# Axionis47/semantic-search-kd

Hardware: AMD Instinct MI355X
Metric: docs embedded/sec + queries/sec@top-10 (1M×384-d corpus), 1→8 MI355X (higher is better)
Workload: dtype bf16 screen + f32 exact; 1 GPU; cosine top-10: 10000 queries x 1000000 x 384-d fp32 corpus in HBM (configs[1] search), row-sharded over 1 GPU(s), all-gather + merge; corpus_rows=1000000, queries=10000, k=10, queries_per_block=160, corpus_passes=63, slices=4, exact_fallback_queries=0, index_bytes=1536000000, sidecar_bytes=768004096, workspace_bytes=697277184

## Files before the change

include/sskd_amd.h:

```cpp
#ifndef SSKD_AMD_H
#define SSKD_AMD_H

#include <stddef.h>
#include <stdint.h>

#ifdef __cplusplus
extern "C" {
#endif

#define SSKD_ABI_VERSION 1

#define SSKD_OK 0
#define SSKD_ERR_INVALID 1
#define SSKD_ERR_WORKSPACE 2
#define SSKD_ERR_HIP 3
#define SSKD_ERR_UNSUPPORTED 4

#define SSKD_DIM 384
#define SSKD_TILE_ROWS 32
#define SSKD_K_PASS 32
#define SSKD_K_MAX 1024

int sskd_abi_version(void);
const char* sskd_last_error(void);
// ... 37 lines not shown

size_t sskd_index_bf16_bytes(int64_t n_rows);
int sskd_index_make_bf16(const float* d_tiled, int64_t n_rows, void* d_bf16, void* stream);
size_t sskd_index_search_screened_workspace_bytes(int64_t n_rows, int nq, int k);
int sskd_index_search_screened_plan(int64_t n_rows, int nq, int k, int* queries_per_block, int* corpus_passes,
                                    int* n_slices);
int sskd_index_search_screened(const float* d_tiled, const void* d_bf16, int64_t n_rows, const float* d_queries,
                               int nq, int k, int64_t id_offset, float* d_out_scores, int64_t* d_out_ids,
                               int* d_status, void* d_workspace, size_t workspace_bytes, void* stream,
                               void* ev_scan_begin, void* ev_scan_end);

size_t sskd_index_screen_band_scratch_bytes(int nq);
int sskd_index_screen_band(const void* d_bf16, int64_t n_rows, const float* d_queries, int nq, float* d_eps2_out,
                           void* d_scratch, size_t scratch_bytes, void* stream);

int sskd_index_screen_scores(const void* d_bf16, int64_t n_rows, const float* d_queries, int nq, float* d_out, void* stream);
int sskd_screen_threshold_roundtrip(const float* d_in, int n, float* d_out, void* stream);

int sskd_index_search_screened_plan_claims(int64_t n_rows, int nq, int k, int* claims);
int sskd_index_search_screened_claim(const float* d_tiled, const void* d_bf16, int64_t n_rows, const float* d_queries,
                                     int nq, int k, int64_t id_offset, const uint32_t* d_row_mask, int claim,
                                     float* d_out_scores, int64_t* d_out_ids, int* d_status, void* d_workspace,
                                     size_t workspace_bytes, void* stream, void* ev_scan_begin, void* ev_scan_end);

size_t sskd_index_search_onepass_workspace_bytes(int64_t n_rows, int nq, int k);
int sskd_index_search_onepass(const float* d_tiled, int64_t n_rows, const float* d_queries, int nq,
                              int k, int64_t id_offset, float* d_out_scores, int64_t* d_out_ids,
                              int* d_inexact, void* d_workspace, size_t workspace_bytes,
                              void* stream);

int64_t sskd_row_mask_words(int64_t n_rows);
int sskd_row_mask_pack(const uint8_t* d_flags, int64_t n_rows, uint32_t* d_mask, void* stream);
int sskd_row_mask_update(uint32_t* d_mask, int64_t n_rows, const int64_t* d_rows, int64_t n_ids, int allow,
                         int* d_bad, void* stream);
int sskd_row_mask_and(const uint32_t* d_a, const uint32_t* d_b, int64_t n_rows, uint32_t* d_out, void* stream);
int sskd_row_mask_count(const uint32_t* d_mask, int64_t n_rows, int64_t* d_count, void* stream);

int sskd_index_search_filtered(const float* d_tiled, int64_t n_rows, const float* d_queries, int nq, int k,
                               int64_t id_offset, const uint32_t* d_row_mask, float* d_out_scores,
                               int64_t* d_out_ids, void* d_workspace, size_t workspace_bytes, void* stream,
                               const sskd_search_tuning* tuning, void* ev_scan_begin, void* ev_scan_end);
int sskd_index_search_screened_filtered(const float* d_tiled, const void* d_bf16, int64_t n_rows, const float* d_queries,
                                        int nq, int k, int64_t id_offset, const uint32_t* d_row_mask, float* d_out_scores,
                                        int64_t* d_out_ids, int* d_status, void* d_workspace, size_t workspace_bytes,
                                        void* stream, void* ev_scan_begin, void* ev_scan_end);
int sskd_index_search_onepass_filtered(const float* d_tiled, int64_t n_rows, const float* d_queries, int nq,
// ... 387 lines not shown
```

semantic-search-kd_amd/_native.py:

```python
from __future__ import annotations

import ctypes as C
from pathlib import Path
from typing import Optional

_LIB_PATH = Path(__file__).resolve().parent / "libsskd_amd.so"

SSKD_OK = 0
SSKD_DIM = 384
SSKD_TILE_ROWS = 32
SSKD_K_PASS = 32
SSKD_K_MAX = 1024

_ERR_NAMES = {1: "INVALID", 2: "WORKSPACE", 3: "HIP", 4: "UNSUPPORTED"}


class NativeError(RuntimeError):

    def __init__(self, code: int, message: str):
        super().__init__(f"sskd_amd[{_ERR_NAMES.get(code, code)}]: {message}")
        self.code = code


class EncoderConfig(C.Structure):
# ... 95 lines not shown
    "sskd_index_search": (_i, [_vp, _i64, _vp, _i, _i, _i64, _vp, _vp, _vp, _sz, _vp]),
    "sskd_index_search_profiled": (_i, [_vp, _i64, _vp, _i, _i, _i64, _vp, _vp, _vp, _sz, _vp, _vp, _vp]),
    "sskd_index_search_plan": (_i, [_i64, _i, _i, _ip, _ip, _ip, _ip, _ip]),
    "sskd_index_search_workspace_bytes_ex": (_sz, [_i64, _i, _i, C.POINTER(SearchTuning)]),
    "sskd_index_search_ex": (
        _i, [_vp, _i64, _vp, _i, _i, _i64, _vp, _vp, _vp, _sz, _vp, C.POINTER(SearchTuning), _vp, _vp]
    ),
    "sskd_index_search_plan_ex": (_i, [_i64, _i, _i, C.POINTER(SearchTuning), _ip, _ip, _ip, _ip, _ip]),
    "sskd_topk_record_bytes": (_sz, [_i, _i]),
    "sskd_topk_merge_packed": (_i, [_vp, _i, _i, _i, _i, _vp, _vp, _vp]),
    "sskd_index_bf16_bytes": (_sz, [_i64]),
    "sskd_index_make_bf16": (_i, [_vp, _i64, _vp, _vp]),
    "sskd_index_search_screened_workspace_bytes": (_sz, [_i64, _i, _i]),
    "sskd_index_search_screened_plan": (_i, [_i64, _i, _i, _ip, _ip, _ip]),
    "sskd_index_search_screened": (_i, [_vp, _vp, _i64, _vp, _i, _i, _i64, _vp, _vp, _vp, _vp, _sz, _vp, _vp, _vp]),
    "sskd_index_search_screened_plan_claims": (_i, [_i64, _i, _i, _ip]),
    "sskd_index_search_screened_claim": (
        _i, [_vp, _vp, _i64, _vp, _i, _i, _i64, _vp, _i, _vp, _vp, _vp, _vp, _sz, _vp, _vp, _vp]
    ),
    "sskd_index_screen_band_scratch_bytes": (_sz, [_i]),
    "sskd_index_screen_band": (_i, [_vp, _i64, _vp, _i, _vp, _vp, _sz, _vp]),
    "sskd_index_screen_scores": (_i, [_vp, _i64, _vp, _i, _vp, _vp]),
    "sskd_screen_threshold_roundtrip": (_i, [_vp, _i, _vp, _vp]),
    "sskd_index_search_onepass_workspace_bytes": (_sz, [_i64, _i, _i]),
    "sskd_index_search_onepass": (_i, [_vp, _i64, _vp, _i, _i, _i64, _vp, _vp, _vp, _vp, _sz, _vp]),
    "sskd_row_mask_words": (_i64, [_i64]),
    "sskd_row_mask_pack": (_i, [_vp, _i64, _vp, _vp]),
    "sskd_row_mask_update": (_i, [_vp, _i64, _vp, _i64, _i, _vp, _vp]),
    "sskd_row_mask_and": (_i, [_vp, _vp, _i64, _vp, _vp]),
    "sskd_row_mask_count": (_i, [_vp, _i64, _vp, _vp]),
    "sskd_index_search_filtered": (
        _i, [_vp, _i64, _vp, _i, _i, _i64, _vp, _vp, _vp, _vp, _sz, _vp, C.POINTER(SearchTuning), _vp, _vp]
    ),
    "sskd_index_search_screened_filtered": (
        _i, [_vp, _vp, _i64, _vp, _i, _i, _i64, _vp, _vp, _vp, _vp, _vp, _sz, _vp, _vp, _vp]
    ),
    "sskd_index_search_onepass_filtered": (_i, [_vp, _i64, _vp, _i, _i, _i64, _vp, _vp, _vp, _vp, _vp, _sz, _vp]),
    "sskd_index_range_search_workspace_bytes": (_sz, [_i64, _i, _i64]),
    "sskd_index_range_search": (_i, [_vp, _i64, _vp, _i, _vp, _i64, _vp, _vp, _vp, _vp, _i64, _vp, _sz, _vp]),
    "sskd_range_record_bytes": (_sz, [_i, _i64]),
    "sskd_range_merge_workspace_bytes": (_sz, [_i, _i, _i64]),
    "sskd_range_merge_packed": (_i, [_vp, _i, _i, _i64, _vp, _vp, _vp, _i64, _vp, _sz, _vp]),
    "sskd_index_search_grouped_workspace_bytes": (_sz, [_i64, _i, _i, _i]),
    "sskd_index_search_grouped": (
        _i, [_vp, _i64, _vp, _i, _i, _i, _i64, _vp, _vp, _vp, _vp, _vp, _vp, _vp, _vp, _vp, _sz, _vp]
    ),
# ... 188 lines not shown
```

semantic-search-kd_amd/csrc/screen.hip:

```cpp
#include "search_device.h"
#include "search_host.h"

#include <algorithm>
#include <cfloat>

using sskd::require_shard_rows;

namespace {

typedef __bf16 sbf16x8 __attribute__((ext_vector_type(8)));
typedef float f32x4 __attribute__((ext_vector_type(4)));
constexpr int BSTEPS = DIM / 32;
constexpr int BTILE_VEC = 2 * BSTEPS * 64;
#ifndef SSKD_SCREEN_BGROUP
#define SSKD_SCREEN_BGROUP 3
#endif
#ifndef SSKD_SCREEN_WAVES
#define SSKD_SCREEN_WAVES 12
#endif
#ifndef SSKD_SCREEN_RING
#define SSKD_SCREEN_RING 2
#endif
constexpr int BGROUP = SSKD_SCREEN_BGROUP;
constexpr int SCREEN_RING = SSKD_SCREEN_RING;
#ifndef SSKD_SCREEN_BGROUP_Q5
#define SSKD_SCREEN_BGROUP_Q5 1
#endif
#ifndef SSKD_SCREEN_RING_Q5
#define SSKD_SCREEN_RING_Q5 3
#endif
constexpr int BGROUP_Q5 = SSKD_SCREEN_BGROUP_Q5, SCREEN_RING_Q5 = SSKD_SCREEN_RING_Q5;
#ifndef SSKD_SCREEN_TAU_REFRESH_TILES
#define SSKD_SCREEN_TAU_REFRESH_TILES 64
#endif
constexpr int SCREEN_TAU_REFRESH_TILES = SSKD_SCREEN_TAU_REFRESH_TILES;
#ifndef SSKD_SCREEN_BOUND_REFRESH_TILES
#define SSKD_SCREEN_BOUND_REFRESH_TILES 8
#endif
constexpr int SCREEN_BOUND_REFRESH_TILES = SSKD_SCREEN_BOUND_REFRESH_TILES;
constexpr int SCREEN_WAVES = SSKD_SCREEN_WAVES;
template <int BG, int RG>
struct ScreenRingOk {
  static_assert(BSTEPS % BG == 0 && (BSTEPS / BG) % RG == 0 && RG >= 2, "screening prefetch geometry");
  static constexpr bool value = true;
};
static_assert(ScreenRingOk<BGROUP, SCREEN_RING>::value && ScreenRingOk<BGROUP_Q5, SCREEN_RING_Q5>::value, "");
constexpr float SCREEN_ACC_SLACK = 1.0e-4f;
constexpr int SCREEN_MAX_CAND = 256;
constexpr int SCREEN_FALLBACK_TIER1 = 1024;
constexpr int SCREEN_LIGHT_MAX_TILES_PER_WAVE = 330;
constexpr int SCREEN_CUS = 256;

__global__ __launch_bounds__(256) void tile_colsum_kernel(const float4* __restrict__ tiled, int64_t n_tiles,
                                                          float* __restrict__ colsum) {
  const int c = threadIdx.x % CHUNKS, g = threadIdx.x / CHUNKS;
  if (g >= 2) return;
  float4 a = make_float4(0.f, 0.f, 0.f, 0.f);
  for (int64_t t = blockIdx.x; t < n_tiles; t += gridDim.x) {
// ... 46 lines not shown
    }
    out[t * BTILE_VEC + v] = o;
    atomicAdd(&rowss[0][r], nn);
    atomicAdd(&rowss[1][r], bb);
    atomicAdd(&rowss[2][r], dd);
    atomicMax(&amax, am);
  }
  __syncthreads();
  if (threadIdx.x < 96) {
    const float v = rowss[threadIdx.x >> 5][threadIdx.x & 31];
    atomicMax(norm_block + (threadIdx.x >> 5), __float_as_int(v < INFINITY ? v : INFINITY));
  }
  if (threadIdx.x == 96) atomicMax(norm_block + SIDECAR_ABSMAX_WORD, amax);
}

constexpr float SCREEN_MIN_CORPUS = 0x1p-40f, SCREEN_MIN_QUERY = 0x1p-96f;
constexpr float SCREEN_MIN_BAND = 0x1p-100f, SCREEN_MAX_BAND = 0x1p+100f;
__global__ __launch_bounds__(256) void screen_setup_kernel(const float* __restrict__ queries, int nq,
                                                           const int* __restrict__ max_norm2, float* __restrict__ eps2,
                                                           int* __restrict__ tau, int* __restrict__ fb_count,
                                                           int* __restrict__ d_status, int* __restrict__ cursors,
                                                           int n_cursors) {
  for (int i = blockIdx.x * 256 + threadIdx.x; i < n_cursors; i += gridDim.x * 256) cursors[i] = 0;
  if (threadIdx.x < 44) {
    const int64_t i = (int64_t)blockIdx.x * 44 + threadIdx.x;
    if (i < (int64_t)nq * 11) tau[i] = (int)0x80000000;
  }
  if (blockIdx.x == 0) {
    if (threadIdx.x < 64) fb_count[threadIdx.x] = 0;
    if (threadIdx.x < 2) d_status[threadIdx.x] = 0;
  }
  const int lane = threadIdx.x & 63;
  const int q = blockIdx.x * 4 + (threadIdx.x >> 6);
  if (q >= nq) return;
  float xs[DIM / 64];
  int am = 0;
#pragma unroll
  for (int i = 0; i < DIM / 64; ++i) {
    xs[i] = queries[(int64_t)q * DIM + lane + 64 * i];
    am = max(am, __float_as_int(xs[i]) & 0x7fffffff);
  }
#pragma unroll
  for (int o = 32; o > 0; o >>= 1) am = max(am, __shfl_xor(am, o));
  const int ex = min(max(am >> 23, 1), 253);
  const float down = __int_as_float(ex << 23), up = __int_as_float((254 - ex) << 23);
  float ss = 0.f, dd = 0.f;
#pragma unroll
  for (int i = 0; i < DIM / 64; ++i) {
    const float x = xs[i];
// ... 230 lines not shown
      for (int nb = 0; nb < 2 * QB; ++nb)
#pragma unroll
        for (int i = 0; i < 4; ++i) acc[mb][nb][i] = 0.f;
    screen_tile_groups<QB, 0, BG, RG, SCREEN_FRAG_DEPTH, NB>(buf, tiled + (int64_t)t * BTILE_VEC, qbase, qfrag, acc,
                                                             t + 1 < n_tiles, (int64_t)BTILE_VEC, lane_off);
#pragma unroll
    for (int mb = 0; mb < 2; ++mb)
#pragma unroll
      for (int nb = 0; nb < 2 * QB; ++nb)
#pragma unroll
        for (int i = 0; i < 4; ++i)
          out[(int64_t)(t * TILE_ROWS + 16 * mb + 4 * g + i) * (32 * QB) + 16 * nb + n] = acc[mb][nb][i];
  }
}

__global__ __launch_bounds__(256) void screen_thr_probe_kernel(const float* __restrict__ in, int n, float* __restrict__ out) {
  const int i = blockIdx.x * 256 + threadIdx.x;
  if (i >= n) return;
  const float x = in[i], y = (i ^ 1) < n ? in[i ^ 1] : -INFINITY;
  const unsigned packed = (i & 1) ? screen_thr_pack2(y, x) : screen_thr_pack2(x, y);
  out[i] = screen_thr_unpack(packed, i & 1);
}

template <int QB>
__device__ __forceinline__ void apply_tile_mask16(f32x4 (&acc)[2][2 * QB], uint32_t word, int g) {
  if (word == 0xFFFFFFFFu) return;
  const uint32_t lw = word >> (4 * g);
#pragma unroll
  for (int mb = 0; mb < 2; ++mb)
#pragma unroll
    for (int i = 0; i < 4; ++i) {
      const bool off = ((lw >> (16 * mb + i)) & 1u) == 0u;
#pragma unroll
      for (int nb = 0; nb < 2 * QB; ++nb)
        if (off) acc[mb][nb][i] = -INFINITY;
    }
}

template <int K, int QB, int WAVES, bool BOUND_ONLY, bool LIGHT, int BG, int RG, bool MASKED = false>
__device__ __forceinline__ void screen_tiles(const ScreenAppendParams& p, int t_begin, int t_end, int slice, int* cursors,
                                             int wave, int n, int g, int q0,
                                             const sbf16x8* __restrict__ qlane, int* pool, int list0,
                                             bool ragged, unsigned (&gthr)[QB]) {
  constexpr int NQ = 2 * QB;
  int* const wthr = pool + QB * 32 * K;
  float* const bandl = reinterpret_cast<float*>(wthr + QB * 32);
  short* const cnts = reinterpret_cast<short*>(bandl + QB * 32);
  sbf16x8 buf[RG][BG][2];
  constexpr int NB = screen_frag_bases<QB>();
  screen_lds_frag* qbase[NB];
#pragma unroll
  for (int nb = 0; nb < NB; ++nb) {
    qbase[nb] = (screen_lds_frag*)qlane + nb * SCREEN_FRAGS_PER_BASE * 64;
    asm volatile("" : "+v"(qbase[nb]));
  }
  sbf16x8 qfrag[SCREEN_FRAG_DEPTH];
#ifdef SSKD_SCREEN_ABL_CONTIG
  const unsigned lane_off = (unsigned)(n + 16 * g) * 16u;
#else
// ... 37 lines not shown
      c_end = next_end;
    }
  }
  if (t >= 0) {
#pragma unroll
    for (int gr = 0; gr + 1 < RG; ++gr) load_bgroup<BG>(buf[gr], p.tiled + (int64_t)t * BTILE_VEC + gr * BG * 128, lane_off);
  }

  for (int tiles_done = 0; t >= 0; t = next_t, ++tiles_done) {
    if (dealt) {
      next_t = t + WAVES < t_end ? t + WAVES : -1;
    } else {
      const int rem = c_end - t;
      if (rem == 2) draw();
      next_t = t + 1;
      if (rem == 1) {
        next_t = drawn_chunk();
        c_end = next_end;
      }
    }
    const sbf16x8* tile = p.tiled + (int64_t)t * BTILE_VEC;
    uint32_t mword = 0xFFFFFFFFu;
    if constexpr (MASKED) mword = tile_mask_word(p.row_mask, t);
    const bool exchange = !BOUND_ONLY && (tiles_done == 0 || tiles_done == 16 || tiles_done % SCREEN_TAU_REFRESH_TILES == 0);
    if (exchange || tiles_done % SCREEN_BOUND_REFRESH_TILES == 0) {
    const int lh = screen_lane_now(), nh = lh & 15;
    if (exchange && lh < 16) {
#pragma unroll
      for (int nb = 0; nb < NQ; ++nb) {
        const int ql = 16 * nb + nh;
        if (q0 + ql < p.nq) atomicMax(wthr + ql, exchange_bound<K>(p.gpool, p.tau + q0 + ql, q0 + ql, wthr[ql]));
      }
    }
#pragma unroll
    for (int pr = 0; pr < QB; ++pr) {
      float thr[2];
#pragma unroll
      for (int e = 0; e < 2; ++e) {
        const int nb = 2 * pr + e, ql = 16 * nb + nh;
        const int w = wthr[ql];
        const float bd = bandl[ql];
        thr[e] = ordered_to_float(w) - bd;
        thr[e] = fmaxf(thr[e], -INFINITY);
      }
      screen_thr_raise2(gthr[pr], thr[0], thr[1]);
      asm volatile("" : "+v"(gthr[pr]));
    }
    }
    f32x4 acc[2][NQ];
#pragma unroll
    for (int mb = 0; mb < 2; ++mb)
#pragma unroll
      for (int nb = 0; nb < NQ; ++nb)
#pragma unroll
        for (int i = 0; i < 4; ++i) acc[mb][nb][i] = 0.f;

// ... 29 lines not shown
      for (int e = 0; e < 2; ++e) {
        const int nb = 2 * pr + e;
        m[e] = acc[0][nb][0];
#pragma unroll
        for (int r = 1; r < 8; ++r) m[e] = fmaxf(m[e], acc[r >> 2][nb][r & 3]);
        fthr[e] = fmaxf(screen_thr_unpack(gthr[pr], e), -FLT_MAX);
        pass[e] = m[e] >= fthr[e];
      }
      if constexpr (BOUND_ONLY) {
#pragma unroll
        for (int e = 0; e < 2; ++e) {
          const int nb = 2 * pr + e;
          const float mg = screen_group_max(pass[e] ? m[e] : -INFINITY);
          if (pass[e]) {
            int nc = n;
            asm volatile("" : "+v"(nc));
            const int ql = 16 * nb + nc;
            if (m[e] == mg) {
              int xid = rowbase;
#pragma unroll
              for (int r = 7; r >= 0; --r) xid = acc[r >> 2][nb][r & 3] == m[e] ? rowbase + 16 * (r >> 2) + (r & 3) : xid;
              const int xi = float_to_ordered(m[e]);
              if (pool_offer<K>(pool + ql * K, wthr + ql, xi)) {
                bucket_forward<K>(p.gpool, q0 + ql, xid, xi);
              }
            }
            screen_thr_raise(gthr[pr], e, fmaxf(ordered_to_float(wthr[ql]) - bandl[ql], -INFINITY));
          }
        }
      } else
      if (__any(pass[0] || pass[1])) {
        const int lc = screen_lane_now(), nc = lc & 15, gc = lc >> 4;
        float pb[2];
        int c[2];
#pragma unroll
        for (int e = 0; e < 2; ++e) {
          const int ql = 32 * pr + 16 * e + nc;
          pb[e] = fmaxf(ordered_to_float(wthr[ql]) - bandl[ql], -INFINITY);
          c[e] = cnts[(ql * WAVES + wave) * 4 + gc];
        }
        screen_thr_raise2(gthr[pr], pb[0], pb[1]);
        const float thr[2] = {fmaxf(pb[0], fthr[0]), fmaxf(pb[1], fthr[1])};
        const auto run_of = [&](int ql) {
          return reinterpret_cast<unsigned long long*>(
              p.cand + ((int64_t)min(q0 + ql, p.nq - 1) * p.lists_per_query + list0 + gc) * SCREEN_CAP);
        };
        const auto compact_if_tight = [&](int ql, int& cc, float bound) {
#ifndef SSKD_SCREEN_NO_COMPACT
          const bool tight = cc > SCREEN_CAP - 8 && cc <= SCREEN_CAP;
          if (__any(tight)) {
            __builtin_amdgcn_s_waitcnt(0x0F70);
            if (tight) cc = screen_compact_run(run_of(ql), cc, bound);
          }
          return tight;
#else
          return false;
#endif
        };
        if constexpr (LIGHT) {
#pragma unroll
// ... 2 lines not shown
            if (!__any(m[e] >= thr[e])) continue;
            unsigned long long* const run = run_of(ql);
            int cc = c[e];
            const bool dirty = compact_if_tight(ql, cc, thr[e]);
            bool grew = false;
#pragma unroll
            for (int r = 0; r < 8; ++r) {
              const float x = acc[r >> 2][nb][r & 3];
              const int xid = rowbase + 16 * (r >> 2) + (r & 3);
              if (x >= thr[e]) {
                if (cc < SCREEN_CAP)
                  run[cc] = (unsigned long long)__float_as_uint(x) | ((unsigned long long)(unsigned)xid << 32);
                if (cc <= SCREEN_CAP) ++cc;
                grew = true;
              }
            }
            if (grew || dirty) cnts[(ql * WAVES + wave) * 4 + gc] = (short)cc;
            const float mg = screen_group_max(m[e]);
            if (grew && m[e] == mg) {
              int xid = rowbase;
#pragma unroll
              for (int r = 7; r >= 0; --r) xid = acc[r >> 2][nb][r & 3] == m[e] ? rowbase + 16 * (r >> 2) + (r & 3) : xid;
              const int xi = float_to_ordered(m[e]);
              if (pool_offer<K>(pool + ql * K, wthr + ql, xi) && tiles_done > 0)
                bucket_forward<K>(p.gpool, q0 + ql, xid, xi);
            }
          }
        } else {
          unsigned take = 0;
#pragma unroll
          for (int b = 15; b >= 0; --b)
            take = (take << 1) | (acc[(b >> 2) & 1][2 * pr + (b >> 3)][b & 3] >= thr[b >> 3] ? 1u : 0u);
          if (!__any(take != 0)) continue;
          int cc[2] = {c[0], c[1]};
          bool dirty[2] = {false, false};
#pragma unroll
          for (int e = 0; e < 2; ++e)
            if (__any((take >> (8 * e) & 0xFFu) != 0)) dirty[e] = compact_if_tight(32 * pr + 16 * e + nc, cc[e], thr[e]);
#pragma clang loop unroll(disable)
          for (unsigned rest = take; rest != 0; rest &= rest - 1) {
            const int b = __builtin_ctz(rest);
            const int e = b >> 3;
            const bool b0 = b & 1, b1 = b & 2, b2 = b & 4, b3 = b & 8;
            const auto &a0 = acc[0][2 * pr], &a1 = acc[1][2 * pr], &a2 = acc[0][2 * pr + 1], &a3 = acc[1][2 * pr + 1];
            const float x00 = b0 ? a0[1] : a0[0], x01 = b0 ? a0[3] : a0[2], x02 = b0 ? a1[1] : a1[0], x03 = b0 ? a1[3] : a1[2];
            const float x04 = b0 ? a2[1] : a2[0], x05 = b0 ? a2[3] : a2[2], x06 = b0 ? a3[1] : a3[0], x07 = b0 ? a3[3] : a3[2];
            const float x10 = b1 ? x01 : x00, x11 = b1 ? x03 : x02, x12 = b1 ? x05 : x04, x13 = b1 ? x07 : x06;
            const float x20 = b2 ? x11 : x10, x21 = b2 ? x13 : x12;
            const float x = b3 ? x21 : x20;
            const int xid = rowbase + 4 * (b & 4) + (b & 3);
            const int ql = 32 * pr + 16 * e + nc;
            int cn = e ? cc[1] : cc[0];
            if (cn < SCREEN_CAP) run_of(ql)[cn] = (unsigned long long)__float_as_uint(x) | ((unsigned long long)(unsigned)xid << 32);
            if (cn <= SCREEN_CAP) ++cn;
            cc[0] = e ? cc[0] : cn;
            cc[1] = e ? cn : cc[1];
            if (tiles_done > 0) {
              const int xi = float_to_ordered(x);
              if (pool_offer<K>(pool + ql * K, wthr + ql, xi))
                bucket_forward<K>(p.gpool, q0 + ql, xid, xi);
            }
          }
#pragma unroll
          for (int e = 0; e < 2; ++e) {
            const int ql = 32 * pr + 16 * e + nc;
            if (!__any((take >> (8 * e) & 0xFFu) != 0)) continue;
            const bool grew = (take >> (8 * e) & 0xFFu) != 0;
            if (grew || dirty[e]) cnts[(ql * WAVES + wave) * 4 + gc] = (short)cc[e];
            if (tiles_done == 0) {
              const float mg = screen_group_max(m[e]);
              if (grew && m[e] == mg) pool_offer<K>(pool + ql * K, wthr + ql, float_to_ordered(m[e]));
            }
          }
        }
      }
    }
  }

}

constexpr size_t screen_lds_bytes(int QB, int WAVES) {
  return (size_t)2 * QB * BSTEPS * 64 * 16 + (size_t)QB * 32 * (10 + 2) * sizeof(int) + (size_t)QB * 32 * WAVES * 4 * sizeof(short);
}
static_assert(screen_lds_bytes(5, SCREEN_WAVES) <= 160 * 1024, "the 160-query workgroup must fit the CU's LDS");

template <int K, int QB, int WAVES, bool LIGHT, int BG, int RG, bool MASKED = false>
__global__ __launch_bounds__(WAVES * 64) void screen_append_kernel(ScreenAppendParams p) {
  static_assert(K == 10, "screen_lds_bytes counts ten pool slots per query");
  extern __shared__ float4 qs_raw[];
  sbf16x8* const qs = reinterpret_cast<sbf16x8*>(qs_raw);
  const int tid = threadIdx.x;
  const int lane = tid & 63;
  const int wave = __builtin_amdgcn_readfirstlane(tid >> 6);
  const int n = lane & 15, g = lane >> 4;
// ... 14 lines not shown
  float* const bandl = reinterpret_cast<float*>(wthr + QB * 32);
  short* const cnts = reinterpret_cast<short*>(bandl + QB * 32);
  for (int i = tid; i < QB * 32 * (K + 1); i += WAVES * 64) pool[i] = (int)0x80000000;
  for (int i = tid; i < QB * 32; i += WAVES * 64) bandl[i] = p.eps2[min(q0 + i, p.nq - 1)];
  for (int i = tid; i < QB * 32 * WAVES * 2; i += WAVES * 64) reinterpret_cast<int*>(cnts)[i] = 0;
  __syncthreads();
  const sbf16x8* qlane = qs + lane;

  unsigned gthr[QB];
#pragma unroll
  for (int pr = 0; pr < QB; ++pr)
    gthr[pr] = (q0 + 32 * pr + n < p.nq ? 0xFC00u : 0x7C00u) | (q0 + 32 * pr + 16 + n < p.nq ? 0xFC000000u : 0x7C000000u);
  const int list0 = (slice * WAVES + wave) * 4;

  const bool ragged = (p.n_rows & 31) != 0;

  const int t_begin = slice * p.tiles_per_slice;
  const int t_end = min(t_begin + p.tiles_per_slice, p.n_tiles);
  if (p.pre_tps > 0) {
    const int s_begin = slice * p.pre_tps;
    const int s_end = min(s_begin + p.pre_tps, p.pre_tiles);
    screen_tiles<K, QB, WAVES, true, LIGHT, BG, RG, MASKED>(p, s_begin, s_end, slice, nullptr, wave, n, g, q0, qlane,
                                             pool, list0, ragged, gthr);
#pragma unroll
    for (int nb = 0; nb < 2 * QB; ++nb)
      if (g == 0 && q0 + nb * 16 + n < p.nq) atomicMax(p.tau + q0 + nb * 16 + n, wthr[nb * 16 + n]);
    __syncthreads();
    if ((SCREEN_STEAL && p.claim) || (s_begin < t_end && t_begin < s_end)) {
      for (int i = tid; i < QB * 32 * K; i += WAVES * 64) pool[i] = (int)0x80000000;
      __syncthreads();
    }
  }
#ifdef SSKD_SCREEN_STAMPS
  if (lane == 0) stamp[1] = __builtin_amdgcn_s_memrealtime();
#endif
  screen_tiles<K, QB, WAVES, false, LIGHT, BG, RG, MASKED>(p, t_begin, t_end, slice, p.cursors + (int64_t)qblk * p.n_slices,
                                            wave, n, g, q0, qlane, pool, list0, ragged, gthr);
#ifdef SSKD_SCREEN_STAMPS
  if (lane == 0) stamp[2] = __builtin_amdgcn_s_memrealtime();
#endif

  const int lt = screen_lane_now(), nt = lt & 15, gt = lt >> 4;
#pragma unroll
  for (int nb = 0; nb < 2 * QB; ++nb) {
    const int q = q0 + nb * 16 + nt;
    if (q < p.nq) p.cand_cnt[(int64_t)q * p.lists_per_query + list0 + gt] = cnts[((nb * 16 + nt) * WAVES + wave) * 4 + gt];
  }
}

struct ScreenFinalAppendParams {
  const uint2* cand;
  const int* cand_cnt;
  const float* eps2;
  const float* rows;
// ... 294 lines not shown
  float* eps2;
  int* fb_count;
  int* cursors;
  int* fb_qid;
  float* fb_queries;
  float* fb_scores;
  int64_t* fb_ids;
  void* exact_ws;
  size_t exact_bytes;
  void* exact_ws2;
  size_t exact_bytes2;
#ifdef SSKD_SCREEN_STAMPS
  unsigned long long* stamps;
#endif
  size_t bytes;
};

ScreenWs screen_carve(void* base, const ScreenPlan& pl, int64_t n_rows, int nq, int k) {
  sskd::Carver c(base);
  ScreenWs w{};
  w.part_scores = c.take<float>(pl.part_elems);
  w.part_ids = c.take<int>(pl.part_elems);
  w.cand_cnt = c.take<int>((size_t)nq * pl.lists_per_query);
  w.tau = c.take<int>((size_t)nq * 11);
  w.eps2 = c.take<float>(nq);
  w.fb_count = c.take<int>(64);
  w.cursors = c.take<int>((size_t)pl.n_qblocks * pl.n_slices);
  w.fb_qid = c.take<int>(nq);
  w.fb_queries = c.take<float>((size_t)nq * DIM);
  w.fb_scores = c.take<float>((size_t)nq * k);
  w.fb_ids = c.take<int64_t>((size_t)nq * k);
  const int tier1 = nq < SCREEN_FALLBACK_TIER1 ? nq : SCREEN_FALLBACK_TIER1;
  w.exact_bytes = sskd::exact_workspace_bytes(n_rows, tier1, k);
  w.exact_ws = c.take<char>(w.exact_bytes);
  w.exact_bytes2 = nq > tier1 ? sskd::exact_workspace_bytes(n_rows, nq - tier1, k) : 0;
  w.exact_ws2 = w.exact_bytes2 ? c.take<char>(w.exact_bytes2) : nullptr;
#ifdef SSKD_SCREEN_STAMPS
  w.stamps = c.take<unsigned long long>((size_t)pl.n_qblocks * pl.n_slices * SCREEN_WAVES * 3);
#endif
  w.bytes = c.bytes();
  return w;
}
}

static inline size_t sidecar_norm_offset(int64_t n_rows) { return (size_t)sskd::ceil_div(n_rows, TILE_ROWS) * BTILE_VEC * 16; }
static inline size_t sidecar_rows_offset(int64_t n_rows) { return sidecar_norm_offset(n_rows) + SIDECAR_NORM_BYTES; }

// ... 8 lines not shown
  return sidecar_rows_offset(n_rows);
}

int sskd_index_make_bf16(const float* d_tiled, int64_t n_rows, void* d_bf16, void* stream) {
  SSKD_REQUIRE(n_rows >= 0, "index_make_bf16: n_rows < 0");
  if (n_rows == 0) return SSKD_OK;
  SSKD_REQUIRE(d_tiled && d_bf16, "index_make_bf16: null pointer");
  hipStream_t st = sskd::as_stream(stream);
  const int64_t tiles = sskd::ceil_div(n_rows, TILE_ROWS);
  int* max_norm2 = reinterpret_cast<int*>(static_cast<char*>(d_bf16) + sidecar_norm_offset(n_rows));
  if (hipMemsetAsync(max_norm2, 0, SIDECAR_NORM_BYTES, st) != hipSuccess) return sskd::fail(SSKD_ERR_HIP, "index_make_bf16: memset failed");
  hipLaunchKernelGGL(tile_colsum_kernel, dim3((unsigned)(tiles < 1024 ? tiles : 1024)), dim3(256), 0, st,
                     reinterpret_cast<const float4*>(d_tiled), tiles, reinterpret_cast<float*>(max_norm2) + SIDECAR_COLSUM_OFF);
  int rc = sskd::check_launch("tile_colsum_kernel");
  if (rc != SSKD_OK) return rc;
  hipLaunchKernelGGL(make_bf16_tiles_kernel, dim3((unsigned)tiles), dim3(256), 0, st,
                     reinterpret_cast<const float4*>(d_tiled), tiles, n_rows, static_cast<sbf16x8*>(d_bf16), max_norm2);
  return sskd::check_launch("make_bf16_tiles_kernel");
}

size_t sskd_index_screen_band_scratch_bytes(int nq) {
  if (nq <= 0) return 0;
  sskd::Carver c(nullptr);
  c.take<int>((size_t)nq * 11);
  c.take<int>(64);
  c.take<int>(2);
  return c.bytes();
}

int sskd_index_screen_band(const void* d_bf16, int64_t n_rows, const float* d_queries, int nq, float* d_eps2_out,
                           void* d_scratch, size_t scratch_bytes, void* stream) {
  SSKD_REQUIRE(n_rows > 0 && nq > 0, "index_screen_band: needs rows and queries (got rows=%lld nq=%d)", (long long)n_rows, nq);
  int rc = require_shard_rows("index_screen_band", n_rows);
  if (rc != SSKD_OK) return rc;
  SSKD_REQUIRE(d_bf16 && d_queries && d_eps2_out, "index_screen_band: null pointer");
  sskd::Carver c(d_scratch);
  int* const tau = c.take<int>((size_t)nq * 11);
  int* const fb_count = c.take<int>(64);
  int* const status = c.take<int>(2);
  if ((rc = sskd::require_workspace("index_screen_band", d_scratch, scratch_bytes, c.bytes())) != SSKD_OK) return rc;
  const int* max_norm2 = reinterpret_cast<const int*>(static_cast<const char*>(d_bf16) + sidecar_norm_offset(n_rows));
  launch_screen_setup(max_norm2, d_queries, nq, d_eps2_out, tau, fb_count, status, nullptr, 0, sskd::as_stream(stream));
  return sskd::check_launch("screen_setup_kernel");
}

int sskd_index_screen_scores(const void* d_bf16, int64_t n_rows, const float* d_queries, int nq, float* d_out, void* stream) {
  SSKD_REQUIRE(n_rows > 0 && nq > 0 && nq <= 64, "index_screen_scores: needs rows and 1..64 queries (got rows=%lld nq=%d)",
               (long long)n_rows, nq);
  int rc = require_shard_rows("index_screen_scores", n_rows);
  if (rc != SSKD_OK) return rc;
  SSKD_REQUIRE(d_bf16 && d_queries && d_out, "index_screen_scores: null pointer");
  const size_t lds = (size_t)2 * 2 * BSTEPS * 64 * 16;
  hipLaunchKernelGGL(screen_scores_probe_kernel, dim3(1), dim3(64), lds, sskd::as_stream(stream),
                     static_cast<const sbf16x8*>(d_bf16), d_queries, nq, (int)sskd::ceil_div(n_rows, TILE_ROWS), d_out);
  return sskd::check_launch("screen_scores_probe_kernel");
}

int sskd_screen_threshold_roundtrip(const float* d_in, int n, float* d_out, void* stream) {
  SSKD_REQUIRE(n >= 0, "screen_threshold_roundtrip: n < 0");
  if (n == 0) return SSKD_OK;
  SSKD_REQUIRE(d_in && d_out, "screen_threshold_roundtrip: null pointer");
  hipLaunchKernelGGL(screen_thr_probe_kernel, dim3((unsigned)sskd::ceil_div(n, 256)), dim3(256), 0, sskd::as_stream(stream),
                     d_in, n, d_out);
  return sskd::check_launch("screen_thr_probe_kernel");
}

int sskd_index_search_screened_plan(int64_t n_rows, int nq, int k, int* queries_per_block, int* corpus_passes,
                                    int* n_slices) {
  ScreenPlan pl{};
  if (!screen_plan(n_rows, nq, k, &pl)) return sskd::fail(SSKD_ERR_UNSUPPORTED, "index_search_screened_plan: shape not served");
  if (queries_per_block) *queries_per_block = 32 * pl.QB;
  if (corpus_passes) *corpus_passes = pl.n_qblocks;
  if (n_slices) *n_slices = pl.n_slices;
  return SSKD_OK;
}

size_t sskd_index_search_screened_workspace_bytes(int64_t n_rows, int nq, int k) {
  ScreenPlan pl{};
  if (!screen_plan(n_rows, nq, k, &pl)) return 0;
  return screen_carve(nullptr, pl, n_rows, nq, k).bytes;
}

int sskd_index_search_screened(const float* d_tiled, const void* d_bf16, int64_t n_rows, const float* d_queries,
                               int nq, int k, int64_t id_offset, float* d_out_scores, int64_t* d_out_ids,
                               int* d_status, void* d_workspace, size_t workspace_bytes, void* stream,
                               void* ev_scan_begin, void* ev_scan_end) {
  return sskd_index_search_screened_filtered(d_tiled, d_bf16, n_rows, d_queries, nq, k, id_offset, nullptr, d_out_scores,
// ... 25 lines not shown
    return sskd::fail(SSKD_ERR_UNSUPPORTED,
                      "index_search_screened: needs k <= 10, nq >= 64 and >= 2048 rows (got k=%d nq=%d rows=%lld): "
                      "use sskd_index_search", k, nq, (long long)n_rows);
  int rc = require_shard_rows("index_search_screened", n_rows);
  if (rc != SSKD_OK) return rc;
  SSKD_REQUIRE(d_tiled && d_bf16 && d_queries && d_out_scores && d_out_ids && d_status,
               "index_search_screened: null pointer");
  if (claim >= 0) pl.claim = claim != 0;
  const ScreenWs w = screen_carve(d_workspace, pl, n_rows, nq, k);
  if ((rc = sskd::require_workspace("index_search_screened", d_workspace, workspace_bytes, w.bytes)) != SSKD_OK) return rc;
  hipStream_t st = sskd::as_stream(stream);
  const int64_t tiles = sskd::ceil_div(n_rows, TILE_ROWS);
  const int* max_norm2 = reinterpret_cast<const int*>(static_cast<const char*>(d_bf16) + sidecar_norm_offset(n_rows));

  launch_screen_setup(max_norm2, d_queries, nq, w.eps2, w.tau, w.fb_count, d_status, w.cursors, pl.n_qblocks * pl.n_slices, st);

  static_assert((4 * SCREEN_WAVES * SCREEN_CAP * sizeof(float)) % 256 == 0, "the runs span part_scores and part_ids back to back");
  ScreenAppendParams sp{};
  sp.tiled = static_cast<const sbf16x8*>(d_bf16);
  sp.queries = d_queries;
  sp.eps2 = w.eps2;
  sp.cand = reinterpret_cast<uint2*>(w.part_scores);
  sp.cand_cnt = w.cand_cnt;
  sp.tau = w.tau;
  sp.gpool = w.tau + nq;
  sp.cursors = w.cursors;
  sp.n_rows = n_rows;
  sp.nq = nq;
  sp.lists_per_query = pl.lists_per_query;
  sp.claim = pl.claim ? 1 : 0;
  sp.row_mask = d_row_mask;
#ifdef SSKD_SCREEN_STAMPS
  sp.stamps = w.stamps;
#endif
  const size_t lds = screen_lds_bytes(pl.QB, SCREEN_WAVES);
  const void* kern = nullptr;
  switch (pl.QB) {
#define SSKD_SCREEN_KERN(qb, light, bg, rg)                                                                           \
  (d_row_mask ? reinterpret_cast<const void*>(screen_append_kernel<10, qb, SCREEN_WAVES, light, bg, rg, true>)       \
              : reinterpret_cast<const void*>(screen_append_kernel<10, qb, SCREEN_WAVES, light, bg, rg>))
#define SSKD_SCREEN_CASE(qb, bg, rg)                                                                                  \
  case qb:                                                                                                            \
    kern = pl.light ? SSKD_SCREEN_KERN(qb, true, bg, rg) : SSKD_SCREEN_KERN(qb, false, bg, rg);                       \
    break;
    SSKD_SCREEN_CASE(2, BGROUP, SCREEN_RING)
    SSKD_SCREEN_CASE(4, BGROUP, SCREEN_RING)
    SSKD_SCREEN_CASE(5, BGROUP_Q5, SCREEN_RING_Q5)
#undef SSKD_SCREEN_CASE
// ... 58 lines not shown
```

semantic-search-kd_amd/csrc/search_device.h:

```cpp
#pragma once
#include "common.h"

typedef float f32x16 __attribute__((ext_vector_type(16)));

namespace {

constexpr int DIM = SSKD_DIM;
constexpr int TILE_ROWS = SSKD_TILE_ROWS;
constexpr int STEPS = DIM / 8;
constexpr int CHUNKS = DIM / 4;
constexpr int TILE_FLOATS = TILE_ROWS * DIM;
constexpr int GROUP = 8;
constexpr int GROUPS = STEPS / GROUP;
constexpr int STEP_FLOATS = 8;
__host__ __device__ inline int tile_idx4(int r, int c) { return r * (DIM / 4) + c; }
__host__ __device__ constexpr int acc_row(int r) { return (r & 3) + 8 * (r >> 2); }

__device__ inline float row_score_fma(const float4* src, const float* qv) {
  float acc = 0.f;
#pragma unroll 16
  for (int u = 0; u < STEPS; ++u) {
    const float4 a = src[2 * u], c = src[2 * u + 1];
    const float4 qa = *reinterpret_cast<const float4*>(&qv[8 * u]), qc = *reinterpret_cast<const float4*>(&qv[8 * u + 4]);
    acc = fmaf(a.x, qa.x, acc); acc = fmaf(c.x, qc.x, acc);
// ... 88 lines not shown
      for (int i = 0; i < K; ++i)
        if (i != mi && v[i] < nm) nm = v[i];
      if (nm != (int)0x80000000) atomicMax(thr, nm);
      return true;
    }
  }
  return false;
}

template <int K>
__device__ __forceinline__ void bucket_forward(int* __restrict__ gpool, int q, int xid, int xi) {
  (void)__hip_atomic_fetch_max(gpool + (int64_t)q * K + xid % K, xi, __ATOMIC_RELAXED, __HIP_MEMORY_SCOPE_AGENT);
}

template <int K>
__device__ __forceinline__ int exchange_bound(const int* __restrict__ gpool, int* tau_q, int q, int w) {
  const int* gb = gpool + (int64_t)q * K;
  int bmin = __hip_atomic_load(&gb[0], __ATOMIC_RELAXED, __HIP_MEMORY_SCOPE_AGENT);
#pragma unroll
  for (int i = 1; i < K; ++i)
    bmin = min(bmin, __hip_atomic_load(&gb[i], __ATOMIC_RELAXED, __HIP_MEMORY_SCOPE_AGENT));
  const int old = atomicMax(tau_q, max(w, bmin));
  return max(old, bmin);
}

typedef const __attribute__((address_space(4))) uint32_t const_u32;
__device__ inline uint32_t tile_mask_word(const uint32_t* __restrict__ row_mask, int t) {
  return ((const_u32*)row_mask)[t];
}
template <int QB>
__device__ inline void apply_tile_mask(f32x16 (&acc)[QB], uint32_t word, int h) {
  if (word == 0xFFFFFFFFu) return;
  const uint32_t lw = word >> (4 * h);
#pragma unroll
  for (int r = 0; r < 16; ++r) {
    const bool off = ((lw >> acc_row(r)) & 1u) == 0u;
#pragma unroll
    for (int qq = 0; qq < QB; ++qq)
      if (off) acc[qq][r] = -INFINITY;
  }
}

__device__ inline void load_group(float4 (&buf)[GROUP], const float* __restrict__ base) {
#pragma unroll
  for (int s = 0; s < GROUP; ++s)
    buf[s] = *reinterpret_cast<const float4*>(base + s * STEP_FLOATS);
// ... 60 lines not shown
```

Baseline: 1.801 million queries/s.

## Widen global bound buckets and tighten screen threshold exchange

The cross-block per-query pool grows from K buckets to 16 buckets keyed by row id. The threshold is now the K-th largest bucket value rather than the bucket minimum, which gives a tighter pruning bound. Exchanges are spread across waves, happen more often (every 16 tiles plus early power-of-two tiles), and run after the prescan for all queries. An early-out skips pool_offer when a candidate cannot beat the current wave threshold. The risks are extra atomic traffic, more frequent exchanges, and a slightly larger workspace.

```diff
diff --git a/include/sskd_amd.h b/include/sskd_amd.h
--- a/include/sskd_amd.h
+++ b/include/sskd_amd.h
@@ -83,6 +83,9 @@
                                      int nq, int k, int64_t id_offset, const uint32_t* d_row_mask, int claim,
                                      float* d_out_scores, int64_t* d_out_ids, int* d_status, void* d_workspace,
                                      size_t workspace_bytes, void* stream, void* ev_scan_begin, void* ev_scan_end);
+
+int sskd_screen_bucket_count(void);
+int sskd_screen_bucket_bound(const int32_t* d_in, int nq, int k, int32_t* d_out, void* stream);
 
 size_t sskd_index_search_onepass_workspace_bytes(int64_t n_rows, int nq, int k);
 int sskd_index_search_onepass(const float* d_tiled, int64_t n_rows, const float* d_queries, int nq,
diff --git a/semantic-search-kd_amd/_native.py b/semantic-search-kd_amd/_native.py
--- a/semantic-search-kd_amd/_native.py
+++ b/semantic-search-kd_amd/_native.py
@@ -141,6 +141,8 @@
     "sskd_index_screen_band": (_i, [_vp, _i64, _vp, _i, _vp, _vp, _sz, _vp]),
     "sskd_index_screen_scores": (_i, [_vp, _i64, _vp, _i, _vp, _vp]),
     "sskd_screen_threshold_roundtrip": (_i, [_vp, _i, _vp, _vp]),
+    "sskd_screen_bucket_count": (_i, []),
+    "sskd_screen_bucket_bound": (_i, [_vp, _i, _i, _vp, _vp]),
     "sskd_index_search_onepass_workspace_bytes": (_sz, [_i64, _i, _i]),
     "sskd_index_search_onepass": (_i, [_vp, _i64, _vp, _i, _i, _i64, _vp, _vp, _vp, _vp, _sz, _vp]),
     "sskd_row_mask_words": (_i64, [_i64]),
diff --git a/semantic-search-kd_amd/csrc/screen.hip b/semantic-search-kd_amd/csrc/screen.hip
--- a/semantic-search-kd_amd/csrc/screen.hip
+++ b/semantic-search-kd_amd/csrc/screen.hip
@@ -31,9 +31,20 @@
 #endif
 constexpr int BGROUP_Q5 = SSKD_SCREEN_BGROUP_Q5, SCREEN_RING_Q5 = SSKD_SCREEN_RING_Q5;
 #ifndef SSKD_SCREEN_TAU_REFRESH_TILES
-#define SSKD_SCREEN_TAU_REFRESH_TILES 64
+#define SSKD_SCREEN_TAU_REFRESH_TILES 16
 #endif
 constexpr int SCREEN_TAU_REFRESH_TILES = SSKD_SCREEN_TAU_REFRESH_TILES;
+#ifndef SSKD_SCREEN_BUCKETS
+#define SSKD_SCREEN_BUCKETS 16
+#endif
+constexpr int SCREEN_BUCKETS = SSKD_SCREEN_BUCKETS;
+static_assert(SCREEN_BUCKETS >= 10 && (SCREEN_BUCKETS & (SCREEN_BUCKETS - 1)) == 0, "a power of two of at least K buckets");
+#ifdef SSKD_SCREEN_NO_OFFER_EARLY_OUT
+constexpr bool SCREEN_OFFER_EARLY_OUT = false;
+#else
+constexpr bool SCREEN_OFFER_EARLY_OUT = true;
+#endif
+constexpr int SCREEN_BOUND_WORDS = SCREEN_BUCKETS + 1;
 #ifndef SSKD_SCREEN_BOUND_REFRESH_TILES
 #define SSKD_SCREEN_BOUND_REFRESH_TILES 8
 #endif
@@ -126,9 +137,9 @@
                                                            int* __restrict__ d_status, int* __restrict__ cursors,
                                                            int n_cursors) {
   for (int i = blockIdx.x * 256 + threadIdx.x; i < n_cursors; i += gridDim.x * 256) cursors[i] = 0;
-  if (threadIdx.x < 44) {
-    const int64_t i = (int64_t)blockIdx.x * 44 + threadIdx.x;
-    if (i < (int64_t)nq * 11) tau[i] = (int)0x80000000;
+  for (int j = threadIdx.x; j < 4 * SCREEN_BOUND_WORDS; j += 256) {
+    const int64_t i = (int64_t)blockIdx.x * (4 * SCREEN_BOUND_WORDS) + j;
+    if (i < (int64_t)nq * SCREEN_BOUND_WORDS) tau[i] = (int)0x80000000;
   }
   if (blockIdx.x == 0) {
     if (threadIdx.x < 64) fb_count[threadIdx.x] = 0;
@@ -405,6 +416,15 @@
   out[i] = screen_thr_unpack(packed, i & 1);
 }
 
+template <int K>
+__global__ __launch_bounds__(256) void screen_bucket_bound_kernel(const int* __restrict__ in, int nq, int* __restrict__ out) {
+  const int q = blockIdx.x * 256 + threadIdx.x;
+  if (q >= nq) return;
+  int v[SCREEN_BUCKETS];
+  bucket_load_wide<SCREEN_BUCKETS>(v, in, q);
+  out[q] = kth_largest<K, SCREEN_BUCKETS>(v);
+}
+
 template <int QB>
 __device__ __forceinline__ void apply_tile_mask16(f32x4 (&acc)[2][2 * QB], uint32_t word, int g) {
   if (word == 0xFFFFFFFFu) return;
@@ -418,6 +438,28 @@
       for (int nb = 0; nb < 2 * QB; ++nb)
         if (off) acc[mb][nb][i] = -INFINITY;
     }
+}
+
+template <int K, int B, int QB, int LANES>
+__device__ __forceinline__ void screen_exchange(const ScreenAppendParams& p, int q0, int l, int* wthr) {
+  constexpr int QPL = (32 * QB + LANES - 1) / LANES;
+  int v[QPL][B], w[QPL], kth[QPL], old[QPL], qa[QPL];
+  bool live[QPL];
+#pragma unroll
+  for (int j = 0; j < QPL; ++j) {
+    const int ql = l + j * LANES;
+    live[j] = ql < 32 * QB && q0 + ql < p.nq;
+    qa[j] = min(q0 + ql % (32 * QB), p.nq - 1);
+    bucket_load_wide<B>(v[j], p.gpool, qa[j]);
+    w[j] = wthr[ql % (32 * QB)];
+  }
+#pragma unroll
+  for (int j = 0; j < QPL; ++j) kth[j] = kth_largest<K, B>(v[j]);
+#pragma unroll
+  for (int j = 0; j < QPL; ++j) old[j] = atomicMax(p.tau + qa[j], live[j] ? max(w[j], kth[j]) : (int)0x80000000);
+#pragma unroll
+  for (int j = 0; j < QPL; ++j)
+    if (live[j]) atomicMax(wthr + l + j * LANES, max(old[j], kth[j]));
 }
 
 template <int K, int QB, int WAVES, bool BOUND_ONLY, bool LIGHT, int BG, int RG, bool MASKED = false>
@@ -501,16 +543,18 @@
     const sbf16x8* tile = p.tiled + (int64_t)t * BTILE_VEC;
     uint32_t mword = 0xFFFFFFFFu;
     if constexpr (MASKED) mword = tile_mask_word(p.row_mask, t);
-    const bool exchange = !BOUND_ONLY && (tiles_done == 0 || tiles_done == 16 || tiles_done % SCREEN_TAU_REFRESH_TILES == 0);
+    bool exchange = false;
+    if constexpr (!BOUND_ONLY) {
+      constexpr int T = SCREEN_TAU_REFRESH_TILES;
+      const bool periodic = tiles_done % T == 0;
+      if (tiles_done > 0 && (periodic || (tiles_done <= 8 && (tiles_done & (tiles_done - 1)) == 0))) {
+        const int x = periodic ? 4 + tiles_done / T : 1 + __builtin_ctz(tiles_done);
+        exchange = x % WAVES == wave;
+      }
+    }
+    if (exchange) screen_exchange<K, SCREEN_BUCKETS, QB, 64>(p, q0, screen_lane_now(), wthr);
     if (exchange || tiles_done % SCREEN_BOUND_REFRESH_TILES == 0) {
-    const int lh = screen_lane_now(), nh = lh & 15;
-    if (exchange && lh < 16) {
-#pragma unroll
-      for (int nb = 0; nb < NQ; ++nb) {
-        const int ql = 16 * nb + nh;
-        if (q0 + ql < p.nq) atomicMax(wthr + ql, exchange_bound<K>(p.gpool, p.tau + q0 + ql, q0 + ql, wthr[ql]));
-      }
-    }
+    const int nh = screen_lane_now() & 15;
 #pragma unroll
     for (int pr = 0; pr < QB; ++pr) {
       float thr[2];
@@ -586,7 +630,7 @@
               for (int r = 7; r >= 0; --r) xid = acc[r >> 2][nb][r & 3] == m[e] ? rowbase + 16 * (r >> 2) + (r & 3) : xid;
               const int xi = float_to_ordered(m[e]);
               if (pool_offer<K>(pool + ql * K, wthr + ql, xi)) {
-                bucket_forward<K>(p.gpool, q0 + ql, xid, xi);
+                bucket_forward_wide<SCREEN_BUCKETS>(p.gpool, q0 + ql, xid, xi);
               }
             }
             screen_thr_raise(gthr[pr], e, fmaxf(ordered_to_float(wthr[ql]) - bandl[ql], -INFINITY));
@@ -596,10 +640,11 @@
       if (__any(pass[0] || pass[1])) {
         const int lc = screen_lane_now(), nc = lc & 15, gc = lc >> 4;
         float pb[2];
-        int c[2];
+        int c[2], wi[2];
 #pragma unroll
         for (int e = 0; e < 2; ++e) {
           const int ql = 32 * pr + 16 * e + nc;
+          wi[e] = SCREEN_OFFER_EARLY_OUT ? wthr[ql] : (int)0x80000000;
           pb[e] = fmaxf(ordered_to_float(wthr[ql]) - bandl[ql], -INFINITY);
           c[e] = cnts[(ql * WAVES + wave) * 4 + gc];
         }
@@ -648,8 +693,8 @@
 #pragma unroll
               for (int r = 7; r >= 0; --r) xid = acc[r >> 2][nb][r & 3] == m[e] ? rowbase + 16 * (r >> 2) + (r & 3) : xid;
               const int xi = float_to_ordered(m[e]);
-              if (pool_offer<K>(pool + ql * K, wthr + ql, xi) && tiles_done > 0)
-                bucket_forward<K>(p.gpool, q0 + ql, xid, xi);
+              if ((!SCREEN_OFFER_EARLY_OUT || xi > wi[e]) && pool_offer<K>(pool + ql * K, wthr + ql, xi) && tiles_done > 0)
+                bucket_forward_wide<SCREEN_BUCKETS>(p.gpool, q0 + ql, xid, xi);
             }
           }
         } else {
@@ -683,8 +728,8 @@
             cc[1] = e ? cn : cc[1];
             if (tiles_done > 0) {
               const int xi = float_to_ordered(x);
-              if (pool_offer<K>(pool + ql * K, wthr + ql, xi))
-                bucket_forward<K>(p.gpool, q0 + ql, xid, xi);
+              if ((!SCREEN_OFFER_EARLY_OUT || xi > (e ? wi[1] : wi[0])) && pool_offer<K>(pool + ql * K, wthr + ql, xi))
+                bucket_forward_wide<SCREEN_BUCKETS>(p.gpool, q0 + ql, xid, xi);
             }
           }
 #pragma unroll
@@ -695,7 +740,7 @@
             if (grew || dirty[e]) cnts[(ql * WAVES + wave) * 4 + gc] = (short)cc[e];
             if (tiles_done == 0) {
               const float mg = screen_group_max(m[e]);
-              if (grew && m[e] == mg) pool_offer<K>(pool + ql * K, wthr + ql, float_to_ordered(m[e]));
+              if (grew && m[e] == mg && (!SCREEN_OFFER_EARLY_OUT || float_to_ordered(m[e]) > wi[e])) pool_offer<K>(pool + ql * K, wthr + ql, float_to_ordered(m[e]));
             }
           }
         }
@@ -756,14 +801,12 @@
     const int s_end = min(s_begin + p.pre_tps, p.pre_tiles);
     screen_tiles<K, QB, WAVES, true, LIGHT, BG, RG, MASKED>(p, s_begin, s_end, slice, nullptr, wave, n, g, q0, qlane,
                                              pool, list0, ragged, gthr);
-#pragma unroll
-    for (int nb = 0; nb < 2 * QB; ++nb)
-      if (g == 0 && q0 + nb * 16 + n < p.nq) atomicMax(p.tau + q0 + nb * 16 + n, wthr[nb * 16 + n]);
     __syncthreads();
     if ((SCREEN_STEAL && p.claim) || (s_begin < t_end && t_begin < s_end)) {
       for (int i = tid; i < QB * 32 * K; i += WAVES * 64) pool[i] = (int)0x80000000;
-      __syncthreads();
-    }
+    }
+    if (tid < 32 * QB) screen_exchange<K, SCREEN_BUCKETS, QB, 32 * QB>(p, q0, tid, wthr);
+    __syncthreads();
   }
 #ifdef SSKD_SCREEN_STAMPS
   if (lane == 0) stamp[1] = __builtin_amdgcn_s_memrealtime();
@@ -1104,7 +1147,7 @@
   w.part_scores = c.take<float>(pl.part_elems);
   w.part_ids = c.take<int>(pl.part_elems);
   w.cand_cnt = c.take<int>((size_t)nq * pl.lists_per_query);
-  w.tau = c.take<int>((size_t)nq * 11);
+  w.tau = c.take<int>((size_t)nq * SCREEN_BOUND_WORDS);
   w.eps2 = c.take<float>(nq);
   w.fb_count = c.take<int>(64);
   w.cursors = c.take<int>((size_t)pl.n_qblocks * pl.n_slices);
@@ -1159,7 +1202,7 @@
 size_t sskd_index_screen_band_scratch_bytes(int nq) {
   if (nq <= 0) return 0;
   sskd::Carver c(nullptr);
-  c.take<int>((size_t)nq * 11);
+  c.take<int>((size_t)nq * SCREEN_BOUND_WORDS);
   c.take<int>(64);
   c.take<int>(2);
   return c.bytes();
@@ -1172,7 +1215,7 @@
   if (rc != SSKD_OK) return rc;
   SSKD_REQUIRE(d_bf16 && d_queries && d_eps2_out, "index_screen_band: null pointer");
   sskd::Carver c(d_scratch);
-  int* const tau = c.take<int>((size_t)nq * 11);
+  int* const tau = c.take<int>((size_t)nq * SCREEN_BOUND_WORDS);
   int* const fb_count = c.take<int>(64);
   int* const status = c.take<int>(2);
   if ((rc = sskd::require_workspace("index_screen_band", d_scratch, scratch_bytes, c.bytes())) != SSKD_OK) return rc;
@@ -1200,6 +1243,26 @@
   hipLaunchKernelGGL(screen_thr_probe_kernel, dim3((unsigned)sskd::ceil_div(n, 256)), dim3(256), 0, sskd::as_stream(stream),
                      d_in, n, d_out);
   return sskd::check_launch("screen_thr_probe_kernel");
+}
+
+int sskd_screen_bucket_count(void) { return SCREEN_BUCKETS; }
+
+int sskd_screen_bucket_bound(const int32_t* d_in, int nq, int k, int32_t* d_out, void* stream) {
+  SSKD_REQUIRE(nq >= 0 && k >= 1 && k <= 10, "screen_bucket_bound: needs nq >= 0 and 1 <= k <= 10 (got nq=%d k=%d)", nq, k);
+  if (nq == 0) return SSKD_OK;
+  SSKD_REQUIRE(d_in && d_out, "screen_bucket_bound: null pointer");
+  SSKD_REQUIRE(reinterpret_cast<uintptr_t>(d_in) % 8 == 0, "screen_bucket_bound: d_in must be 8-byte aligned");
+  const dim3 grid((unsigned)sskd::ceil_div(nq, 256)), block(256);
+  hipStream_t st = sskd::as_stream(stream);
+  switch (k) {
+#define SSKD_BUCKET_BOUND_CASE(kk) \
+  case kk: hipLaunchKernelGGL(screen_bucket_bound_kernel<kk>, grid, block, 0, st, d_in, nq, d_out); break;
+    SSKD_BUCKET_BOUND_CASE(1) SSKD_BUCKET_BOUND_CASE(2) SSKD_BUCKET_BOUND_CASE(3) SSKD_BUCKET_BOUND_CASE(4)
+    SSKD_BUCKET_BOUND_CASE(5) SSKD_BUCKET_BOUND_CASE(6) SSKD_BUCKET_BOUND_CASE(7) SSKD_BUCKET_BOUND_CASE(8)
+    SSKD_BUCKET_BOUND_CASE(9) SSKD_BUCKET_BOUND_CASE(10)
+#undef SSKD_BUCKET_BOUND_CASE
+  }
+  return sskd::check_launch("screen_bucket_bound_kernel");
 }
 
 int sskd_index_search_screened_plan(int64_t n_rows, int nq, int k, int* queries_per_block, int* corpus_passes,
@@ -1271,8 +1334,8 @@
   sp.eps2 = w.eps2;
   sp.cand = reinterpret_cast<uint2*>(w.part_scores);
   sp.cand_cnt = w.cand_cnt;
-  sp.tau = w.tau;
-  sp.gpool = w.tau + nq;
+  sp.gpool = w.tau;
+  sp.tau = w.tau + (size_t)nq * SCREEN_BUCKETS;
   sp.cursors = w.cursors;
   sp.n_rows = n_rows;
   sp.nq = nq;
diff --git a/semantic-search-kd_amd/csrc/search_device.h b/semantic-search-kd_amd/csrc/search_device.h
--- a/semantic-search-kd_amd/csrc/search_device.h
+++ b/semantic-search-kd_amd/csrc/search_device.h
@@ -134,6 +134,42 @@
     bmin = min(bmin, __hip_atomic_load(&gb[i], __ATOMIC_RELAXED, __HIP_MEMORY_SCOPE_AGENT));
   const int old = atomicMax(tau_q, max(w, bmin));
   return max(old, bmin);
+}
+
+template <int B>
+__device__ __forceinline__ void bucket_forward_wide(int* __restrict__ gpool, int q, int xid, int xi) {
+  (void)__hip_atomic_fetch_max(gpool + (int64_t)q * B + (unsigned)xid % B, xi, __ATOMIC_RELAXED, __HIP_MEMORY_SCOPE_AGENT);
+}
+
+template <int B>
+__device__ __forceinline__ void bucket_load_wide(int (&v)[B], const int* __restrict__ gpool, int q) {
+  static_assert(B % 2 == 0, "two bucket words per load");
+  const unsigned long long* gb = reinterpret_cast<const unsigned long long*>(gpool + (int64_t)q * B);
+#pragma unroll
+  for (int i = 0; i < B / 2; ++i) {
+    const unsigned long long w = __hip_atomic_load(gb + i, __ATOMIC_RELAXED, __HIP_MEMORY_SCOPE_AGENT);
+    v[2 * i] = (int)(unsigned)w;
+    v[2 * i + 1] = (int)(unsigned)(w >> 32);
+  }
+}
+
+template <int K, int B>
+__device__ __forceinline__ int kth_largest(const int (&v)[B]) {
+  static_assert(K >= 1 && K <= B, "K-th largest of B words");
+  int top[K];
+#pragma unroll
+  for (int i = 0; i < K; ++i) top[i] = (int)0x80000000;
+#pragma unroll
+  for (int j = 0; j < B; ++j) {
+    int x = v[j];
+#pragma unroll
+    for (int i = 0; i < K && i <= j; ++i) {
+      const int hi = max(top[i], x);
+      x = min(top[i], x);
+      top[i] = hi;
+    }
+  }
+  return top[K - 1];
 }
 
 typedef const __attribute__((address_space(4))) uint32_t const_u32;
```

Result: faster. 1.868 million queries/s, median of 6 (+3.7%).
